# YufengJin/BundleSDF

Hardware: AMD Instinct MI355X
Metric: NeRF training rays/sec + ms/iter, 64-frame pool, 2048 rays/frame (higher is better)
Workload: dtype fp16 table+MLP (MFMA) / fp32 accumulate+Adam (amp)

## Files before the change

### bundlesdf_amd/csrc/field_step.hip

```cpp
#include <array>
#include <vector>

#include "field_core.h"
#include "field_host.h"

#pragma clang fp contract(off)

namespace nof {

constexpr int LOSS_ACC_COUNTERS = 136;
constexpr int LOSS_ACC_WORDS = 144;
constexpr int TREC = 12;
enum { TR_WSUM = 0, TR_NVALID, TR_LFS, TR_LEM, TR_LSDF, TR_CNT, TR_RACC = 8, TR_LFSR = 11 };
enum { TC_SIG = 1, TC_COL = 2, TC_CRCOL = 4, TC_CRSIG = 8 };
constexpr int LOSS_COPIES = 64, LOSS_SLOTS = 16, LOSS_FOLD_N = 13;
constexpr uint64_t LOSS_ZERO_WORDS = 16 + (uint64_t)LOSS_COPIES * LOSS_SLOTS;

template <int CTRL> __device__ __forceinline__ int dpp_i(int v) {
    return __builtin_amdgcn_update_dpp(0, v, CTRL, 0xf, 0xf, true);
}
#define DPP_ROW_SHL(n) (0x100 + (n))
#define DPP_ROW_SHR(n) (0x110 + (n))

constexpr uint32_t SLOT_EMPTY = 0xffffffffu;
// ... 545 lines not shown
__device__ __forceinline__ void stage_block(const FieldArgs &a, char *smem) {
    NOF_STAGE_FRAGS(TM, NFR, FR0, false, a, smem, (staged_bias<TM, NFR>(smem)));
    __syncthreads();
}

template <typename TM, int WPB, int WAVES, bool DBG>
__global__ __launch_bounds__(WPB * 64) __attribute__((amdgpu_waves_per_eu(WAVES, WAVES))) void k_colour(FieldArgs a_) {
    const FieldArgs a = step_args(a_);
    const int wave = threadIdx.x >> 6, lane = threadIdx.x & 63;
    const int n = lane & 31, h = lane >> 5;
    extern __shared__ __attribute__((aligned(16))) char smem[];
    stage_block<TM, COL_NFR, COL_FR0>(a, smem);
    const float *s_b = staged_bias<TM, COL_NFR>(smem);
    LdsWt<TM> W(reinterpret_cast<const TM *>(smem), lane, COL_FR0);
    const int n_col = __builtin_amdgcn_readfirstlane(a.n_tiles[1]);
    const int wg = __builtin_amdgcn_readfirstlane((int)blockIdx.x * WPB + wave);
    const int stride = gridDim.x * WPB;
    typedef typename FragT<TM>::T Frag;
    int cur = wg < n_col ? a.ctile_list[wg] : 0;
    int nxt = a.ctile_list[min(wg + stride, max(n_col - 1, 0))];
    Frag cin_n;
    frag_zero<TM>(cin_n);
    float z_n = 0.f;
    auto fetch = [&](int sid_first) {
        z_n = a.zbuf[(size_t)sid_first + n];
        cin_n = load_cin<TM>(a.tile_aux + (size_t)(sid_first >> 5) * TILE_AUX, lane);
    };
    if (wg < n_col) fetch(__builtin_amdgcn_readfirstlane(cur));
    __builtin_amdgcn_s_waitcnt(0x0f70);
    for (int li = wg; li < n_col; li += stride) {
        const int sid0 = __builtin_amdgcn_readfirstlane(cur);
        const int nn = a.ctile_list[min(li + 2 * stride, n_col - 1)];
        const int r = sid0 / a.S;
        const size_t slot = (size_t)(sid0 >> 5);
        const size_t sid = (size_t)sid0 + n;
        const RayCtx c = load_ray(a, r);
        const float z = z_n;
        const float w = bell_weight(a, c.depth, z);
        float p[3], x[3];
        const bool valid = sample_point(c, z, p, x);
        const bool front = z < c.depth - a.trunc;
        float wc = valid && w > 0.f ? w : 0.f;
        float wf = a.fs_rgb_w > 0.f && front && valid && c.rtype == 0 ? a.inv_3RS : 0.f;
        asm volatile("" : "+v"(wc), "+v"(wf));
        const Frag shf = sh_frag<TM>(c, h, a.n_ff);
        Acts<TM> A;
        float logit[3];
        W.fence();
        mlp_colour_net_cin<TM>(W, s_b, A, cin_n, shf, lane, logit);
        fetch(__builtin_amdgcn_readfirstlane(li + stride < n_col ? nxt : sid0));
        float rc[3], lf = 0.f;
#pragma unroll
        for (int cc = 0; cc < 3; ++cc) {
            const float sg = sigmoidf(logit[cc]);
            rc[cc] = wc * sg;
            lf += (sg - 1.f) * (sg - 1.f) * wf;
        }
        if constexpr (DBG) {
            if (h == 0) {
                float *o = a.dbg_raw + sid * 4;
                o[0] = logit[0]; o[1] = logit[1]; o[2] = logit[2];
            }
        }
        if constexpr (sizeof(TM) == 2) {
            reinterpret_cast<h8v *>(a.tile_aux + slot * TILE_AUX + 192)[lane] = shf;
            float vx, vy, vz;
            view_dir(c, vx, vy, vz);
            const float2 d = lane == 0 ? make_float2(c.vd[0], c.vd[1])
                                       : (lane == 1 ? make_float2(c.vd[2], vx) : make_float2(vy, vz));
            reinterpret_cast<float2 *>(a.tile_aux + slot * TILE_AUX + min(lane, 2))[1] = d;
        }
        float s0, s1, s2, sf;
        half_sums(h == 0 ? rc[0] : rc[1], s0, s1);
        half_sums(h == 0 ? rc[2] : lf, s2, sf);
        reinterpret_cast<float4 *>(a.rrec + slot * TREC)[2] = make_float4(s0, s1, s2, sf);
        cur = nxt;
        nxt = nn;
    }
}

__global__ __launch_bounds__(256) void k_ray_final(FieldArgs a_) {
    const FieldArgs a = step_args(a_);
    const int r = blockIdx.x * blockDim.x + threadIdx.x;
    const int lane = threadIdx.x & 63, wave = threadIdx.x >> 6;
    float v[10];
#pragma unroll
    for (int k = 0; k < 10; ++k) v[k] = 0.f;
    if (r < a.R) {
        const int ntiles = a.S / 32;
        float wtot = 0.f, nvalid = 0.f, lfs = 0.f, lem = 0.f, lsdf = 0.f, lfsr = 0.f;
        float racc[3] = {0.f, 0.f, 0.f};
        int csig = 0, ccol = 0, crcol = 0, crsig = 0;
#pragma unroll 4
        for (int t = 0; t < ntiles; ++t) {
            const size_t slot = (size_t)r * ntiles + t;
            const float4 *q = reinterpret_cast<const float4 *>(a.rrec + slot * TREC);
            const float4 q0 = q[0], q1 = q[1], q2 = q[2];
            const uint8_t fl = a.tile_bwd[slot];
            wtot += q0.x; nvalid += q0.y; lfs += q0.z; lem += q0.w; lsdf += q1.x;
            const int cnt = __float_as_int(q1.y);
            csig += cnt & TC_SIG; ccol += (cnt >> 1) & 1; crcol += (cnt >> 2) & 1; crsig += (cnt >> 3) & 1;
            if (fl == 1 || fl == 3) {
                racc[0] += q2.x; racc[1] += q2.y; racc[2] += q2.z; lfsr += q2.w;
            }
        }
        const float *cx = a.rctx + (size_t)r * RCTX;
        const float tgt[3] = {cx[3], cx[4], cx[5]};
        const int frame = __float_as_int(cx[23]), rtype = __float_as_int(cx[24]);
        const bool vray = nvalid > 0.f && rtype == 0;
        const float rw = vray ? (frame == 0 ? a.ffw : 1.f) : 0.f;
        float drgb[3], lr = 0.f, rgb[3];
#pragma unroll
        for (int cc = 0; cc < 3; ++cc) {
            rgb[cc] = racc[cc] / (wtot + 1e-10f);
            const float e = rgb[cc] - tgt[cc];
            drgb[cc] = a.rgb_w * 2.f * e * rw * a.inv_3R;
            lr += e * e * rw;
        }
        v[0] = a.rgb_w * lr * a.inv_3R;
        v[1] = lfs * rw;
        v[2] = lem * rw;
        v[3] = lsdf * rw;
        v[4] = nvalid;
        v[5] = lfsr * rw;
        v[6] = (float)csig; v[7] = (float)ccol; v[8] = (float)crcol; v[9] = (float)crsig;
        if (a.dbg_rgb) {
            a.dbg_rgb[r * 3] = rgb[0]; a.dbg_rgb[r * 3 + 1] = rgb[1]; a.dbg_rgb[r * 3 + 2] = rgb[2];
        }
        float4 *ra = reinterpret_cast<float4 *>(a.ray_aux + (size_t)r * RAY_AUX);
        ra[0] = make_float4(drgb[0], drgb[1], drgb[2], wtot);
        ra[1] = make_float4(rw, 0.f, 0.f, 0.f);
        float4 *rg = reinterpret_cast<float4 *>(a.ray_grad + (size_t)r * 12);
        rg[0] = make_float4(0.f, 0.f, 0.f, 0.f);
        rg[1] = make_float4(0.f, 0.f, 0.f, 0.f);
        rg[2] = make_float4(0.f, 0.f, 0.f, 0.f);
    }
    __shared__ float s_v[4][10];
#pragma unroll
    for (int k = 0; k < 10; ++k) {
        const float t = wave_sum(v[k]);
        if (lane == 0) s_v[wave][k] = t;
    }
    __syncthreads();
    if (threadIdx.x < 10) {
        const int k = threadIdx.x;
        const float t = s_v[0][k] + s_v[1][k] + s_v[2][k] + s_v[3][k];
        constexpr int slot[10] = {0, 1, 2, 3, 4, 10, 6, 7, 8, 9};
        if (t != 0.f && (k != 5 || a.fs_rgb_w > 0.f)) atomic_add_f32(loss_row(a, (int)blockIdx.x) + slot[k], t);
    }
}

constexpr int ENCODE_GROUP_SMALL = 2;

constexpr int COMPACT_PER_BLOCK = 4096;
__global__ __launch_bounds__(256) void k_compact(const uint8_t *__restrict__ flags, int n, int *__restrict__ list,
                                                 int *__restrict__ count, int per_block, int *__restrict__ clist) {
    __shared__ int s_wave[3][4];
    __shared__ int s_base[3];
    const int lane = threadIdx.x & 63, wave = threadIdx.x >> 6;
    const int fpt = per_block >> 8;
    const int b0 = blockIdx.x * per_block + threadIdx.x * fpt;
    uint8_t fl[16];
    if (fpt == 16 && b0 + 16 <= n) {
        const uint4 v = *reinterpret_cast<const uint4 *>(flags + b0);
        const uint32_t w[4] = {v.x, v.y, v.z, v.w};
#pragma unroll
        for (int k = 0; k < 16; ++k) fl[k] = (uint8_t)(w[k >> 2] >> (8 * (k & 3)));
    } else {
#pragma unroll
        for (int k = 0; k < 16; ++k) fl[k] = (k < fpt && b0 + k < n) ? flags[b0 + k] : 0;
    }
    int mine[3] = {0, 0, 0};
#pragma unroll
    for (int k = 0; k < 16; ++k) {
        mine[0] += fl[k] == 1;
        mine[1] += fl[k] == 2;
        mine[2] += (fl[k] == 1 || fl[k] == 3);
    }
    int pm[3] = {mine[0], mine[1], mine[2]};
#pragma unroll
    for (int o = 1; o < 64; o <<= 1) {
#pragma unroll
        for (int q = 0; q < 3; ++q) {
            const int u = __shfl_up(pm[q], o, 64);
            if (lane >= o) pm[q] += u;
        }
    }
    if (lane == 63) {
#pragma unroll
        for (int q = 0; q < 3; ++q) s_wave[q][wave] = pm[q];
    }
    __syncthreads();
    if (threadIdx.x < 3) {
        const int q = threadIdx.x;
        const int tot = s_wave[q][0] + s_wave[q][1] + s_wave[q][2] + s_wave[q][3];
        int *cnt = count + (q == 0 ? 0 : (q == 1 ? 2 : 1));
        s_base[q] = (tot && (q < 2 || clist)) ? atomicAdd(cnt, tot) : 0;
    }
    __syncthreads();
    int off[3];
#pragma unroll
    for (int q = 0; q < 3; ++q) {
        off[q] = s_base[q] + pm[q] - mine[q];
        for (int w = 0; w < wave; ++w) off[q] += s_wave[q][w];
    }
#pragma unroll
    for (int k = 0; k < 16; ++k) {
        const int i = b0 + k;
        if (fl[k] == 1) list[off[0]++] = i << 5;
        if (fl[k] == 2) list[n - 1 - off[1]++] = (i << 5) | (int)0x80000000;
        if (clist && (fl[k] == 1 || fl[k] == 3)) clist[off[2]++] = i << 5;
    }
}

__device__ __forceinline__ int bwd_entry(const FieldArgs &a, int li, int n_c, int cap) {
    return a.tile_sid[li < n_c ? li : cap - 1 - (li - n_c)];
}

#include "field_mlp_bwd.h"

__device__ __forceinline__ void loss_fold(const float *__restrict__ part, float *__restrict__ loss_acc, int k) {
    if (k >= LOSS_FOLD_N) return;
    constexpr int dst[LOSS_FOLD_N] = {0, 1, 2, 3, 4, 5, LOSS_ACC_COUNTERS, LOSS_ACC_COUNTERS + 1, LOSS_ACC_COUNTERS + 2,
                                      LOSS_ACC_COUNTERS + 3, LOSS_ACC_COUNTERS + 4, LOSS_ACC_COUNTERS + 5,
                                      LOSS_ACC_COUNTERS + 6};
    float s = 0.f;
    for (int c = 0; c < LOSS_COPIES; ++c) s += part[c * LOSS_SLOTS + k];
    loss_acc[dst[k]] += s;
}

__host__ __device__ constexpr uint32_t scatter_wave_words(uint32_t mask, int VW) {
    return (1 + VW) * (mask + 1) + 160;
}
template <typename TM, typename TT, bool F16V, int WAVES>
__global__ __launch_bounds__(256) __attribute__((amdgpu_num_sgpr(80), amdgpu_waves_per_eu(WAVES, 8))) void k_scatter(FieldArgs a_) {
    const FieldArgs a = step_args(a_);
    extern __shared__ __attribute__((aligned(16))) char smem[];
    const int lane = threadIdx.x & 63;
    const int wave = __builtin_amdgcn_readfirstlane((int)(threadIdx.x >> 6));
    if (blockIdx.x == 0 && wave == 0) loss_fold(a.loss_part, a.loss_acc, lane);
    const int bx = (a.xcd_order & 2) ? xcd_block(blockIdx.x, gridDim.x) : (int)blockIdx.x;
    const int lpw = a.scatter_lpw, ngrp = ((int)a.L + lpw - 1) / lpw;
    const int gw = __builtin_amdgcn_readfirstlane(bx * 4 + wave);
    const int r = __builtin_amdgcn_readfirstlane(gw / ngrp);
    if (r >= a.R || ABL(65536)) return;
    const int lv0 = __builtin_amdgcn_readfirstlane((gw - r * ngrp) * lpw);
    const int nlev = min(lpw, (int)a.L - lv0);
    const int ntiles = a.S / 32;
    const uint8_t *flags = a.tile_bwd + (size_t)r * ntiles;
    const uint8_t fl = lane < ntiles ? flags[lane] : (uint8_t)0;
    uint32_t gm = lane < ntiles ? a.tile_gmask[(size_t)r * ntiles + lane] : 0u;
    const bool tf = fl == 1 || fl == 2;
    if (!__any(tf) || ABL(131072)) return;
    gm = tf ? gm : 0u;
    const uint32_t mask = a.slot_mask;
    constexpr int VW = F16V ? 1 : 2;
    uint32_t *keys = reinterpret_cast<uint32_t *>(smem) + (size_t)wave * scatter_wave_words(mask, VW);
    uint32_t *vals = F16V ? keys + 1 : keys + mask + 1;
    uint16_t *slist = reinterpret_cast<uint16_t *>(keys + (1 + VW) * (mask + 1));
    if constexpr (F16V) {
        for (uint32_t s = lane; s <= mask; s += 64) reinterpret_cast<uint2 *>(keys)[s] = make_uint2(0xffffffffu, 0u);
    } else {
        for (uint32_t s = lane; s <= mask; s += 64) keys[s] = 0xffffffffu;
        for (uint32_t s = lane; s < VW * (mask + 1); s += 64) vals[s] = 0u;
    }
    if ABL(262144) return;
    float *g32 = (sizeof(TM) == 2) ? nullptr : a.grad_table;
    __half *g16 = (sizeof(TM) == 2) ? a.grad_table16 : nullptr;
    const RayCtx c = load_ray(a, r);
    int n_act = 0;
    for (int ch = 0; ch * 64 < a.S; ++ch) {
        const int s = 64 * ch + lane;
        const uint32_t m0 = (uint32_t)__builtin_amdgcn_readlane((int)gm, 2 * ch);
        const uint32_t m1 = 2 * ch + 1 < 64 ? (uint32_t)__builtin_amdgcn_readlane((int)gm, 2 * ch + 1) : 0u;
        const bool cand = s < a.S && (((lane < 32 ? m0 : m1) >> (s & 31)) & 1u);
        const uint64_t b = __ballot(cand);
        if (cand) slist[n_act + (int)__popcll(b & ((1ull << lane) - 1ull))] = (uint16_t)s;
        n_act += (int)__popcll(b);
    }
    n_act = __builtin_amdgcn_readfirstlane(n_act);
    if (n_act == 0) return;
    __builtin_amdgcn_fence(__ATOMIC_SEQ_CST, "wavefront");
    const int nch = (n_act + 63) / 64;
    float sgz[3] = {0.f, 0.f, 0.f}, sg[3] = {0.f, 0.f, 0.f};
    int n_flush = 0, n_direct = 0;
    if (!ABL(32)) {
        typedef typename std::conditional<sizeof(TM) == 2, uint32_t, float2>::type GPair;
        const size_t RS = (size_t)a.R * a.S;
        const int n_it = nlev * nch;
        auto issue = [&](int lv, int ch, float &z, GPair &g, uint32_t &prt) {
            const int j = 64 * ch + lane;
            const int sj_raw = (int)slist[j];
            const int sj = j < n_act ? sj_raw : 0;
            const size_t sid = (size_t)r * a.S + sj;
            prt = sj >= a.N_oct ? 1u : 0u;
            z = a.zbuf[sid];
            g = reinterpret_cast<const GPair *>(a.dfeat)[(size_t)lv * RS + sid];
        };
        float z_nx = 0.f;
        GPair g_nx{};
        uint32_t prt_nx = 0u;
        issue(lv0, 0, z_nx, g_nx, prt_nx);
        int lv = lv0, ch = 0, lv_n = lv0, ch_n = 0;
        for (int it = 0; it < n_it; ++it) {
            const float z = z_nx;
            const GPair gq = g_nx;
            const uint32_t part = prt_nx;
            if (++ch_n == nch) { ch_n = 0; ++lv_n; }
            issue(min(lv_n, (int)a.L - 1), ch_n, z_nx, g_nx, prt_nx);
            const bool member = 64 * ch + lane < n_act;
            float p[3], x[3], g0, g1;
            h2v g01;
            sample_point(load_ray<true>(a, r), z, p, x);
            if constexpr (sizeof(TM) == 2) {
                g01 = __builtin_bit_cast(h2v, gq);
                g0 = (float)g01[0];
                g1 = (float)g01[1];
            } else {
                g01 = h2v{(_Float16)0.f, (_Float16)0.f};
                g0 = gq.x;
                g1 = gq.y;
            }
            const bool act = member && (g0 != 0.f || g1 != 0.f);
            if (ABL(1 << 25)) {
                n_flush += __any(act) ? (int)__popcll(__ballot(act)) : 0;
                n_direct += (__any(act) && lane == 0) ? 64 : 0;
            }
            const bool skipq = ABL(ABL_SKIPQ(lv >> 2));
            if (__any(act) && !skipq) {
                const LevelInfo li = level_info_uniform(a, lv);
                const float x01[3] = {(x[0] + 1) / 2, (x[1] + 1) / 2, (x[2] + 1) / 2};
                float gx[3] = {0.f, 0.f, 0.f};
                backward_level<TT, F16V>(a, li, member, act, part, x01, g0, g1, g01, gx, lane, keys, vals, mask, g32, g16,
                                         n_direct);
#pragma unroll
                for (int i = 0; i < 3; ++i) {
                    sgz[i] = __builtin_fmaf(gx[i], z, sgz[i]);
                    sg[i] += gx[i];
                }
            }
            if (ch == nch - 1 && !ABL(1) && !ABL(1 << 22) && !skipq) {
                const int nfl = flush_table<F16V>(keys, vals, mask, lane, g32, g16, ABL(128));
                n_flush += nfl;
            }
            if (++ch == nch) { ch = 0; ++lv; }
        }
    }
    if (!a.no_dx) {
        float tz[3], t1[3];
#pragma unroll
        for (int i = 0; i < 3; ++i) {
            tz[i] = 0.5f * wave_sum(sgz[i]);
            t1[i] = 0.5f * wave_sum(sg[i]);
        }
        if (lane < 12) {
            const int i = lane >> 2, j = lane & 3;
            const float gzi = i == 0 ? tz[0] : (i == 1 ? tz[1] : tz[2]);
            const float g1i = i == 0 ? t1[0] : (i == 1 ? t1[1] : t1[2]);
            const float dj = j == 0 ? c.dir[0] : (j == 1 ? c.dir[1] : c.dir[2]);
            const float v = j < 3 ? gzi * dj : g1i;
            if (ngrp == 1) a.ray_grad[(size_t)r * 12 + lane] += v;
            else atomic_add_f32(a.ray_grad + (size_t)r * 12 + lane, v);
        }
    }
    if (!a.count_atomics || ABL(16384)) return;
    const float nf = (float)__builtin_amdgcn_readfirstlane(n_flush), nd = wave_sum((float)n_direct);
    float *cnt = a.loss_acc + 8 + 2 * (r & 63);
    if (lane == 0 && nf != 0.f) atomic_add_f32(cnt, nf);
    if (lane == 0 && nd != 0.f) atomic_add_f32(cnt + 1, nd);
}

__global__ __launch_bounds__(256) void k_quad_mirror(FieldArgs a) {
    __shared__ uint32_t s_off[16], s_rs[16], s_end[16];
    if (threadIdx.x < a.L) {
        const LevelInfo li = level_info(a, threadIdx.x);
        s_off[threadIdx.x] = li.off;
        s_rs[threadIdx.x] = li.res + 1;
        s_end[threadIdx.x] = level_dense(li.res + 1, li.hs) ? li.off + li.hs : 0u;
    }
    __syncthreads();
    uint32_t end = 0;
    for (int l = 0; l < (int)a.L && s_end[l]; ++l) end = s_end[l];
    const uint32_t *t = reinterpret_cast<const uint32_t *>(a.table);
    uint4 *quads = const_cast<uint4 *>(a.quads);
    int lv = 0;
    for (uint32_t i = blockIdx.x * 256u + threadIdx.x; i < end; i += gridDim.x * 256u) {
        while (lv + 1 < (int)a.L && s_off[lv + 1] <= i) ++lv;
        const uint32_t rs = s_rs[lv], hi = i + rs + 1;
        if (hi >= s_end[lv]) continue;
        quads[i] = make_uint4(t[i], t[i + 1], t[i + rs], t[hi]);
    }
}

__global__ void k_zero_i32(int *__restrict__ p, int n) {
    const int i = blockIdx.x * blockDim.x + threadIdx.x;
    if (i < n) p[i] = 0;
}

__global__ __launch_bounds__(256) void k_trace(const float *__restrict__ pool, const int32_t *__restrict__ ids, int R,
// ... 56 lines not shown
        bias[i - n_frag_elems] = k >= 0 ? mlp[k] : 0.f;
    }
}

constexpr int SAMPLE_BATCH_MAX = 4096;
__global__ __launch_bounds__(1024) void k_sample_batch(const int64_t *__restrict__ frame_start, int F,
                                                      int rays_per_frame, uint32_t seed, int32_t *__restrict__ ids,
                                                      const nof_step_params *__restrict__ sp) {
    if (sp) seed = sp->batch_seed;
    __shared__ float s_t[1024];
    const int f = blockIdx.x, t = threadIdx.x;
    const int k = rays_per_frame, m = k + 1;
    const int chunk = (m + 1023) / 1024;
    const int j0 = t * chunk, j1 = min(m, j0 + chunk);
    const int64_t lo = frame_start[f], cnt = frame_start[f + 1] - lo;
    float e[5];
    float run = 0.f;
#pragma unroll
    for (int q = 0; q < 5; ++q) {
        e[q] = 0.f;
        const int j = j0 + q;
        if (q < chunk && j < j1) {
            const uint32_t i = (uint32_t)(f * m + j);
            const uint32_t u = hash32(seed ^ hash32(i * 0x85EBCA6BU + 0x27D4EB2FU));
            e[q] = -__logf(((float)u + 0.5f) * 2.3283064e-10f);
            run += e[q];
        }
    }
    s_t[t] = run;
    __syncthreads();
    for (int off = 1; off < 1024; off <<= 1) {
        const float x = s_t[t] + (t >= off ? s_t[t - off] : 0.f);
        __syncthreads();
        s_t[t] = x;
        __syncthreads();
    }
    const float total = s_t[1023];
    float acc = t > 0 ? s_t[t - 1] : 0.f;
    const float scale = (float)cnt / total;
#pragma unroll
    for (int q = 0; q < 5; ++q) {
        const int j = j0 + q;
        if (q < chunk && j < min(j1, k)) {
            acc += e[q];
            int64_t id = (int64_t)(acc * scale);
            id = (id < 0 || cnt <= 0) ? 0 : (id >= cnt ? cnt - 1 : id);
            ids[(size_t)f * k + j] = (int32_t)(lo + id);
        }
    }
}

}

extern "C" int nof_trace_rays(const float *pool, const int32_t *ids, int32_t R, const float *tf, const uint8_t *occ,
                              int32_t N, int32_t Kmax, float near_sc, float far_sc, float trunc, float *rays_out,
                              float *intervals, float *totals, int32_t *counts, const nof_step_params *sp,
                              void *stream) {
    if (R <= 0) return NOF_OK;
    if (N <= 0 || Kmax <= 0) return nof::set_error(NOF_EINVAL, "trace_rays: bad N=%d Kmax=%d", N, Kmax);
    const int tb = R >= 65536 ? 256 : 64;
    hipLaunchKernelGGL(nof::k_trace, dim3(nof::div_up(R, tb)), dim3(tb), 0, (hipStream_t)stream, pool, ids, R, tf,
                       occ, N, Kmax, near_sc, far_sc, trunc, rays_out, intervals, totals, counts, sp,
                       (const int32_t *)nullptr);
    return nof::check_launch("trace_rays");
}

extern "C" int nof_trace_rays_epoch(const float *pool, const int32_t *perm, const int32_t *epoch_step0, int32_t R,
                                    const float *tf, const uint8_t *occ, int32_t N, int32_t Kmax, float near_sc,
                                    float far_sc, float trunc, float *rays_out, float *intervals, float *totals,
                                    int32_t *counts, const nof_step_params *sp, void *stream) {
    if (R <= 0) return NOF_OK;
    if (!perm || !epoch_step0 || !sp)
        return nof::set_error(NOF_EINVAL, "trace_rays_epoch: perm, epoch_step0 and the step block are required");
    if (N <= 0 || Kmax <= 0) return nof::set_error(NOF_EINVAL, "trace_rays_epoch: bad N=%d Kmax=%d", N, Kmax);
    const int tb = R >= 65536 ? 256 : 64;
    hipLaunchKernelGGL(nof::k_trace, dim3(nof::div_up(R, tb)), dim3(tb), 0, (hipStream_t)stream, pool, perm, R, tf,
                       occ, N, Kmax, near_sc, far_sc, trunc, rays_out, intervals, totals, counts, sp, epoch_step0);
    return nof::check_launch("trace_rays_epoch");
}

extern "C" int nof_pack_mlp(const float *mlp, const int32_t *idx, int32_t n_frag_elems, int32_t n_bias, void *frags,
                            float *bias, int mlp_dtype, void *stream) {
    const int n = n_frag_elems + n_bias;
    if (mlp_dtype == NOF_F16)
        hipLaunchKernelGGL(nof::k_pack_mlp<_Float16>, dim3(nof::div_up(n, 256)), dim3(256), 0, (hipStream_t)stream,
                           mlp, idx, n_frag_elems, n_bias, (_Float16 *)frags, bias);
    else
        hipLaunchKernelGGL(nof::k_pack_mlp<float>, dim3(nof::div_up(n, 256)), dim3(256), 0, (hipStream_t)stream, mlp,
                           idx, n_frag_elems, n_bias, (float *)frags, bias);
    return nof::check_launch("pack_mlp");
}

extern "C" int nof_sample_batch(const int64_t *frame_start, int32_t F, int32_t rays_per_frame, uint32_t seed,
                                int32_t *ids, const nof_step_params *sp, void *stream) {
    const int n = F * rays_per_frame;
    if (n <= 0) return NOF_OK;
    if (rays_per_frame > nof::SAMPLE_BATCH_MAX)
        return nof::set_error(NOF_EINVAL, "sample_batch: rays_per_frame %d > %d", rays_per_frame,
                              nof::SAMPLE_BATCH_MAX);
    hipLaunchKernelGGL(nof::k_sample_batch, dim3(F), dim3(1024), 0, (hipStream_t)stream, frame_start,
                       F, rays_per_frame, seed, ids, sp);
    return nof::check_launch("sample_batch");
}

namespace {
constexpr int N_FIELD_KERNELS = 4;
struct FieldTiming {
    bool on = false;
    std::vector<std::array<hipEvent_t, N_FIELD_KERNELS + 1>> sets;
    size_t used = 0;
};
FieldTiming g_timing;
hipEvent_t *timing_set() {
    if (!g_timing.on) return nullptr;
    if (g_timing.used == g_timing.sets.size()) {
        std::array<hipEvent_t, N_FIELD_KERNELS + 1> e{};
        for (auto &x : e)
            if (hipEventCreate(&x) != hipSuccess) return nullptr;
        g_timing.sets.push_back(e);
    }
    return g_timing.sets[g_timing.used++].data();
}
inline void mark(hipEvent_t *ev, int i, hipStream_t st) {
    if (ev) (void)hipEventRecord(ev[i], st);
}

template <typename TM, typename TT, bool DBG>
auto encode_kernel(int g) {
    return g == 4 ? nof::k_encode<TM, TT, 4, DBG> : (g == 2 ? nof::k_encode<TM, TT, 2, DBG> : nof::k_encode<TM, TT, 1, DBG>);
}

template <typename TM, typename TT, int WPB>
int launch_field(const nof::FieldArgs &a, int n_cu, hipStream_t st) {
    const int ntiles = a.S / 32;
    hipLaunchKernelGGL(nof::k_ray_ctx, dim3(nof::div_up(a.R, 256)), dim3(256), 0, st, a);
    hipEvent_t *ev = timing_set();
    mark(ev, 0, st);
    if (a.quads && !a.quads_ready)
        hipLaunchKernelGGL(nof::k_quad_mirror, dim3(nof::tile_blocks(a.n_rows, 256, n_cu, 8)), dim3(256), 0, st, a);
    const size_t elds = (size_t)8 * 64 * 8 * sizeof(TM) + 2 * 64 * sizeof(float) + 8 * 16 * 32;
    {
        const dim3 eg(nof::div_up((uint64_t)a.R * ntiles, 8));
        const bool dbg = a.dbg_z || a.dbg_valid || a.dbg_raw;
        hipLaunchKernelGGL((dbg ? encode_kernel<TM, TT, true>(a.encode_group) : encode_kernel<TM, TT, false>(a.encode_group)),
                           eg, dim3(512), elds, st, a);
    }
    int rc = nof::check_launch("field_step(encode)");
    if (rc) return rc;
    mark(ev, 1, st);
    {
        const int nflags = a.R * ntiles;
        const int per = a.compact_per > 0 ? a.compact_per : (nflags >= 262144 ? nof::COMPACT_PER_BLOCK : 512);
        hipLaunchKernelGGL(nof::k_compact, dim3(nof::div_up((uint64_t)nflags, per)), dim3(256), 0, st, a.tile_bwd,
                           nflags, a.tile_sid, a.n_tiles, per, a.ctile_list);
        rc = nof::check_launch("field_step(compact)");
        if (rc) return rc;
        constexpr int WPB_C = 4;
        const int nbc = std::max(1, nof::tile_blocks(nflags, 8, n_cu, 6));
        const size_t clds = nof::staged_bytes<TM, nof::COL_NFR>();
        hipLaunchKernelGGL((a.dbg_raw ? nof::k_colour<TM, WPB_C, 6, true> : nof::k_colour<TM, WPB_C, 6, false>), dim3(nbc),
                           dim3(WPB_C * 64), clds, st, a);
        rc = nof::check_launch("field_step(colour)");
        if (rc) return rc;
        hipLaunchKernelGGL(nof::k_ray_final, dim3(nof::div_up(a.R, 256)), dim3(256), 0, st, a);
        rc = nof::check_launch("field_step(ray_final)");
        if (rc) return rc;
    }
    mark(ev, 2, st);
    const size_t mlds = nof::staged_bytes<TM, nof::N_FRAGS>(false, 16 * sizeof(float));
    if constexpr (sizeof(TM) == 2) {
        const int64_t nt_all = (int64_t)a.R * ntiles;
        const bool blk = a.bwd_flush != 1;
        const int nbt = std::max(1, nof::tile_blocks(nt_all, blk ? 48 : 128, n_cu, 1));
        const size_t tl0 = nof::bwd_tr_lds(0, 8), tl1 = nof::bwd_tr_lds(1, 8);
        const auto tr0 = a.n_ff > 0 ? (blk ? nof::k_mlp_bwd_tr<8, 0, true, true> : nof::k_mlp_bwd_tr<8, 0, true>)
                                    : (blk ? nof::k_mlp_bwd_tr<8, 0, false, true> : nof::k_mlp_bwd_tr<8, 0>);
        hipLaunchKernelGGL(tr0, dim3(nbt), dim3(8 * 64), tl0, st, a);
        rc = nof::check_launch("field_step(mlp_bwd_tr0)");
        if (rc) return rc;
        hipLaunchKernelGGL((blk ? nof::k_mlp_bwd_tr<8, 1, false, true> : nof::k_mlp_bwd_tr<8, 1>), dim3(nbt), dim3(8 * 64), tl1, st, a);
        rc = nof::check_launch("field_step(mlp_bwd_tr1)");
        if (rc) return rc;
    } else {
        const int nbb = std::max(1, nof::tile_blocks((int64_t)a.R * ntiles, 64, n_cu, 2));
        hipLaunchKernelGGL((nof::k_mlp_bwd<TM, 4, 2, 0>), dim3(nbb), dim3(4 * 64), mlds, st, a);
        rc = nof::check_launch("field_step(mlp_bwd0)");
        if (rc) return rc;
        const int nb1 = std::min(nbb, n_cu);
        hipLaunchKernelGGL((a.n_ff > 0 ? nof::k_mlp_bwd<TM, 4, 1, 1, true> : nof::k_mlp_bwd<TM, 4, 1, 1>), dim3(nb1), dim3(4 * 64), mlds, st, a);
        rc = nof::check_launch("field_step(mlp_bwd)");
        if (rc) return rc;
    }
    mark(ev, 3, st);
    const int n_grp = ((int)a.L + a.scatter_lpw - 1) / a.scatter_lpw;
    const dim3 sg(nof::div_up((uint64_t)a.R * n_grp, 4));
    if constexpr (sizeof(TM) == 2) {
        const size_t lds = (size_t)4 * 4 * nof::scatter_wave_words(a.slot_mask, 1);
        hipLaunchKernelGGL((nof::k_scatter<TM, TT, true, 7>), sg, dim3(256), lds, st, a);
    } else {
        hipLaunchKernelGGL((nof::k_scatter<TM, TT, false, 1>), sg, dim3(256),
                           (size_t)4 * 4 * nof::scatter_wave_words(a.slot_mask, 2), st, a);
    }
    rc = nof::check_launch("field_step(scatter)");
    if (rc) return rc;
    mark(ev, 4, st);
    return NOF_OK;
}

struct FieldWorkspace : nof::Carver {
    void *feat, *dfeat;
    float *zbuf, *ray_aux, *rctx, *rrec;
    uint8_t *tile_bwd;
    int *tile_sid, *n_tiles, *ctile;
    float4 *tile_aux;
    uint32_t *gmask;
    uint64_t off[NOF_WS_SECTIONS] = {};
    template <int I, typename T> T *part(size_t count) {
        static_assert(I < NOF_WS_SECTIONS - 1, "a new section needs a larger NOF_WS_SECTIONS in include/nof.h");
        return off[I] = bytes, take<T>(count);
    }
    FieldWorkspace(void *base, int R, int S, int mlp_dtype) : Carver(base) {
        const size_t el = mlp_dtype == NOF_F16 ? 2 : 4, n = (size_t)R * S, nt = (size_t)R * (S / 32);
        feat = part<0, char>(n * 32 * el);
        dfeat = part<1, char>(n * 32 * el);
        zbuf = part<2, float>(n);
        tile_bwd = part<3, uint8_t>(nt);
        tile_sid = part<4, int>(nt);
        n_tiles = part<5, int>(nof::LOSS_ZERO_WORDS);
        ray_aux = part<6, float>((size_t)R * nof::RAY_AUX);
        tile_aux = part<7, float4>(nt * nof::TILE_AUX);
        rctx = part<8, float>((size_t)R * nof::RCTX);
        gmask = part<9, uint32_t>(nt);
        rrec = part<10, float>(nt * nof::TREC);
        ctile = part<11, int>(nt);
        off[NOF_WS_SECTIONS - 1] = bytes;
    }
};
bool quads_on(const nof_field_desc *d) {
    return d->table_quads && d->table_rows > 0 && d->mlp_dtype == NOF_F16 && d->table_dtype == NOF_F16 &&
           d->R >= (d->quads_min_rays > 0 ? d->quads_min_rays : 32768) && !ABL_HOST(d, 512);
}
}

extern "C" size_t nof_field_workspace_bytes(int32_t R, int32_t S, int32_t mlp_dtype) {
    return FieldWorkspace(nullptr, R, S, mlp_dtype).bytes;
}

extern "C" int nof_field_workspace_offsets(int32_t R, int32_t S, int32_t mlp_dtype, uint64_t *offsets, int32_t n) {
    if (R < 0 || S <= 0 || !offsets || n < NOF_WS_SECTIONS)
        return nof::set_error(NOF_EINVAL, "field_workspace_offsets: bad R=%d S=%d or n=%d < %d", R, S, n,
                              NOF_WS_SECTIONS);
    const FieldWorkspace w(nullptr, R, S, mlp_dtype);
    for (int i = 0; i < NOF_WS_SECTIONS; ++i) offsets[i] = w.off[i];
    return NOF_OK;
}

extern "C" size_t nof_field_desc_size(void) { return sizeof(nof_field_desc); }

extern "C" int nof_quad_mirror(const nof_field_desc *d, void *stream) {
    if (!d) return nof::set_error(NOF_EINVAL, "quad_mirror: desc is NULL");
    if (d->L > 16 || d->C != 2)
        return nof::set_error(NOF_EINVAL, "quad_mirror: needs C=2, L<=16 (got %u,%u)", d->C, d->L);
    if (d->R <= 0 || !quads_on(d)) return NOF_OK;
    nof::FieldArgs a{};
    a.table = d->table; a.levels = (const float4 *)d->levels; a.L = d->L;
    a.quads = (const uint4 *)d->table_quads; a.n_rows = (uint32_t)d->table_rows;
    hipLaunchKernelGGL(nof::k_quad_mirror, dim3(nof::tile_blocks(a.n_rows, 256, nof::cu_count(), 8)), dim3(256), 0,
                       (hipStream_t)stream, a);
    return nof::check_launch("quad_mirror");
}

extern "C" int nof_field_step(const nof_field_desc *d, void *stream) {
    if (!d) return nof::set_error(NOF_EINVAL, "field_step: desc is NULL");
    if (d->S % 32 != 0 || d->S > 320 || d->N_oct + d->N_dep != d->S)
        return nof::set_error(NOF_EINVAL, "field_step: S=%d must be N_oct+N_dep, a multiple of 32, <= 320", d->S);
    if (int rc = nof::check_geometry("field_step", d, false)) return rc;
    if (d->R <= 0) return NOF_OK;
    if (d->bwd_flush < 0 || d->bwd_flush > 2)
        return nof::set_error(NOF_EINVAL, "field_step: bwd_flush %d (0 by batch size, 1 per wave, 2 block)", d->bwd_flush);
    if (d->compact_per_block != 0 && (d->compact_per_block < 256 || d->compact_per_block > nof::COMPACT_PER_BLOCK ||
                                      d->compact_per_block % 256 != 0))
        return nof::set_error(NOF_EINVAL, "field_step: compact_per_block %d (0 by batch size, else a multiple of 256 "
                              "in [256, %d])", d->compact_per_block, nof::COMPACT_PER_BLOCK);
    if (d->encode_group != 0 && d->encode_group != 1 && d->encode_group != 2 && d->encode_group != 4)
        return nof::set_error(NOF_EINVAL, "field_step: encode_group %d (0 by batch size, or 1, 2, 4)", d->encode_group);
    if (int rc = nof::check_frame_features("field_step", d->n_ff, d->ff, d->grad_ff, true)) return rc;
    if (d->mlp_dtype == NOF_F16 && !d->grad_table16)
        return nof::set_error(NOF_EINVAL, "field_step: amp mode needs grad_table16 (fp16 table gradient)");
    if (d->ablate && !NOF_ABLATE)
        return nof::set_error(NOF_EINVAL, "field_step: ablate bits need a -DNOF_ABLATE=1 build (timing experiments only)");
    if (!d->workspace) return nof::set_error(NOF_EINVAL, "field_step: workspace is NULL (nof_field_workspace_bytes)");
    const int slots = d->scatter_slots ? d->scatter_slots : 512;
    if (slots < 64 || slots > 2048 || (slots & (slots - 1)))
        return nof::set_error(NOF_EINVAL, "field_step: scatter_slots must be a power of two in [64, 2048]");
    bool amp;
    if (int rc = nof::check_dtype_pair("field_step", d, amp)) return rc;

    nof::FieldArgs a;
    nof::fill_sampling(a, d);
    nof::fill_model(a, d);
    a.t_rand = d->t_rand; a.seed = d->seed; a.perturb = d->perturb;
    a.fs_sdf = d->fs_sdf; a.ffw = d->first_frame_weight;
    a.rgb_w = d->rgb_weight; a.fs_w = d->fs_weight; a.empty_w = d->empty_weight; a.trunc_w = d->trunc_weight;
    a.inv_3R = 1.0f / (3.0f * (float)d->R);
    a.inv_RS = 1.0f / ((float)d->R * (float)d->S);
    a.inv_3RS = 1.0f / (3.0f * (float)d->R * (float)d->S);
    a.xcd_order = d->xcd_order;
    a.no_dx = d->skip_pose_grad != 0;
    a.quads = quads_on(d) ? (const uint4 *)d->table_quads : nullptr;
    a.n_rows = (uint32_t)d->table_rows;
    a.quads_ready = d->quads_prebuilt != 0;
    {
        const int L = std::max(1, (int)d->L);
        const int want = d->R >= 196608 ? 16 : (d->R >= 32768 ? 8 : (d->R >= 8192 ? 4 : 2));
        a.scatter_lpw = std::max(1, std::min(L, d->scatter_levels_per_wave > 0 ? (int)d->scatter_levels_per_wave : want));
    }
    a.bwd_flush = d->bwd_flush;
    a.count_atomics = d->count_atomics != 0;
    a.compact_per = d->compact_per_block;
    a.encode_group = d->encode_group ? d->encode_group : (d->R >= 8192 ? 1 : nof::ENCODE_GROUP_SMALL);
    a.sp = d->step_params;
    a.fs_rgb_w = d->fs_rgb_weight;
    a.loss_scale = d->loss_scale; a.grad_ff = d->grad_ff;
    a.grad_table = d->grad_table; a.grad_mlp = d->grad_mlp;
    a.grad_table16 = (__half *)d->grad_table16;
    a.ray_grad = d->ray_grad; a.loss_acc = d->loss_acc; a.dbg_z = d->dbg_z; a.dbg_raw = d->dbg_raw;
    a.dbg_valid = d->dbg_valid; a.dbg_rgb = d->dbg_rgb; a.ablate = d->ablate;
    a.slot_mask = (uint32_t)slots - 1;
    const FieldWorkspace ws(d->workspace, d->R, d->S, d->mlp_dtype);
    a.feat = ws.feat; a.dfeat = ws.dfeat; a.zbuf = ws.zbuf; a.tile_bwd = ws.tile_bwd; a.tile_sid = ws.tile_sid;
    a.n_tiles = ws.n_tiles; a.loss_part = (float *)ws.n_tiles + 16;
    a.ray_aux = ws.ray_aux; a.tile_aux = ws.tile_aux; a.rctx = ws.rctx; a.tile_gmask = ws.gmask; a.rrec = ws.rrec;
    a.ctile_list = ws.ctile;

    hipStream_t st = (hipStream_t)stream;
    const int n_cu = nof::cu_count();
    return amp ? launch_field<_Float16, __half, 4>(a, n_cu, st) : launch_field<float, float, 4>(a, n_cu, st);
}

extern "C" int nof_field_timing(int32_t enable) {
    g_timing.on = enable != 0;
    g_timing.used = 0;
    return NOF_OK;
}

extern "C" int nof_field_timing_collect(float *ms_sum, int32_t n, int32_t *calls) {
    if (!ms_sum || n < N_FIELD_KERNELS) return nof::set_error(NOF_EINVAL, "field_timing_collect: need 4 floats");
    for (int k = 0; k < n; ++k) ms_sum[k] = 0.f;
    for (size_t i = 0; i < g_timing.used; ++i) {
        auto &e = g_timing.sets[i];
        if (hipEventSynchronize(e[N_FIELD_KERNELS]) != hipSuccess)
            return nof::set_error(NOF_ELAUNCH, "field_timing_collect: event sync failed");
        for (int k = 0; k < N_FIELD_KERNELS; ++k) {
            float ms = 0.f;
            if (hipEventElapsedTime(&ms, e[k], e[k + 1]) != hipSuccess)
                return nof::set_error(NOF_ELAUNCH, "field_timing_collect: elapsed time failed");
            ms_sum[k] += ms;
        }
    }
    if (calls) *calls = (int32_t)g_timing.used;
    g_timing.used = 0;
    return NOF_OK;
}
```

### bundlesdf_amd/fused.py

```python
import ctypes
import dataclasses
import gc
import math
import os

import numpy as np
import torch

from . import _lib
from . import exchange as EX
from . import mlp_layout as ML

_F32, _F16 = 0, 1
MAX_LEVEL_RES = 1023
QUADS_MIN_RAYS = 32768
MAX_POSE_FRAMES = 1024


def lr_at(cfg, global_step, base):
    n_iters = cfg["n_step"] + 1
    if global_step <= 10:
        return base
    last = 10 * ((global_step - 1) // 10)
    return base * (cfg["decay_rate"] ** (float(last) / n_iters))
# ... 692 lines not shown
                      workspace=torch.empty(int(_lib.lib().nof_render_workspace_bytes(n, S)), dtype=torch.uint8,
                                            device=d))
            self._render_buf = rb
        return rb

    @torch.no_grad()
    def render_rays(self, ids, global_step=None, samples=False, chunk=32768):
        cfg = self.cfg
        ids = torch.as_tensor(ids).to(self.dev).to(torch.int32).contiguous().view(-1)
        R = int(ids.numel())
        S = cfg["N_samples"] + cfg["N_samples_around_depth"]
        dev = self.dev
        out = {"rgb": torch.empty(R, 3, device=dev), "depth": torch.empty(R, device=dev)}
        if samples:
            out.update(z=torch.empty(R, S, device=dev), sdf=torch.empty(R, S, device=dev),
                       valid=torch.empty(R, S, dtype=torch.uint8, device=dev))
        if R > 0:
            chunk = max(1, int(chunk))
            L = _lib.lib()
            st = _lib.stream_of(self.P)
            self.wait_exchange()
            self._prologue()
            sc = cfg["sc_factor"]
            trunc = truncation(cfg, self.global_step if global_step is None else global_step)
            rb = self._render_buffers(min(chunk, R))
            for lo in range(0, R, chunk):
                n = min(chunk, R - lo)
                _lib.check(L.nof_trace_rays(_lib.ptr(self.pool), _lib.ctypes.c_void_p(ids.data_ptr() + 4 * lo), n,
                                            _lib.ptr(self.tf_buf), _lib.ptr(self.occ), self.Nocc, self.Kmax,
                                            cfg["near"] * sc, cfg["far"] * sc, trunc, _lib.ptr(rb["rays"]),
                                            _lib.ptr(rb["intervals"]), _lib.ptr(rb["totals"]), None, None, st),
                           "trace_rays")
                D = _lib.FieldDesc()
                D.R, D.L, D.C, D.D = n, self.L, self.C, 3
                D.table = (self.emb16 if self.amp else self.P).data_ptr()
                D.levels = self.levels.data_ptr()
                D.table_dtype = D.mlp_dtype = _F16 if self.amp else _F32
                D.rays, D.tf, D.intervals, D.totals = (rb["rays"].data_ptr(), self.tf_buf.data_ptr(),
                                                       rb["intervals"].data_ptr(), rb["totals"].data_ptr())
                D.Kmax, D.N_oct, D.N_dep, D.S = self.Kmax, cfg["N_samples"], cfg["N_samples_around_depth"], S
                D.near_sc, D.far_sc, D.trunc = cfg["near"] * sc, cfg["far"] * sc, trunc
                D.neg_trunc_ratio, D.sdf_lambda = cfg["neg_trunc_ratio"], cfg["sdf_lambda"]
                D.frags, D.bias = self.frags.data_ptr(), self.bias.data_ptr()
                D.n_ff = self.n_ff
                if self.n_ff:
                    D.ff = self.P.data_ptr() + 4 * self.feat_off
                O = _lib.RenderOut(rgb=out["rgb"].data_ptr() + 12 * lo, depth=out["depth"].data_ptr() + 4 * lo,
                                   workspace=rb["workspace"].data_ptr())
                if samples:
                    O.z, O.sdf = out["z"].data_ptr() + 4 * S * lo, out["sdf"].data_ptr() + 4 * S * lo
                    O.valid = out["valid"].data_ptr() + S * lo
                _lib.check(L.nof_render_rays(_lib.ctypes.byref(D), _lib.ctypes.byref(O), st), "render_rays")
        if samples:
            out["valid"] = out["valid"].bool()
        return out

    @torch.no_grad()
    def render_view(self, c2w, K, H, W, frame_id=0, step=None, max_steps=512, n_refine=8, pixels=None, chunk=65536,
                    stats=False):
        from .view import pixel_indices
        H, W = int(H), int(W)
        dev = self.dev
        pix = None if pixels is None else pixel_indices(H, W, pixels).to(torch.int32).to(dev).contiguous()
        n = H * W if pix is None else int(pix.numel())
        shape = (H, W) if pix is None else (n,)
        if step is None:
            step = 0.5 * truncation(self.cfg, self.global_step)
        out = {"t": torch.empty(n, device=dev), "depth": torch.empty(n, device=dev),
               "normal": torch.empty(n, 3, device=dev), "rgb": torch.empty(n, 3, device=dev),
               "hit": torch.empty(n, dtype=torch.uint8, device=dev)}
        if stats:
            out.update(index=torch.empty(n, dtype=torch.int32, device=dev),
                       tiles=torch.empty(n, dtype=torch.int32, device=dev))
        V = _lib.ViewDesc()
        V.c2w[:] = np.asarray(c2w, np.float64).astype(np.float32).reshape(16).tolist()
        V.K[:] = np.asarray(K, np.float64).astype(np.float32).reshape(9).tolist()
        V.H, V.W = H, W
        V.step, V.max_steps, V.n_refine = float(step), int(max_steps), int(n_refine)
        V.frame_id, V.n_frames = int(frame_id), self.F
        V.occ, V.occ_n = self.occ.data_ptr(), self.Nocc
        D = _lib.FieldDesc()
        D.L, D.C, D.D, D.Kmax = self.L, self.C, 3, self.Kmax
        D.table = (self.emb16 if self.amp else self.P).data_ptr()
        D.levels = self.levels.data_ptr()
        D.table_dtype = D.mlp_dtype = _F16 if self.amp else _F32
        D.frags, D.bias = self.frags.data_ptr(), self.bias.data_ptr()
        D.n_ff = self.n_ff
        if self.n_ff:
            D.ff = self.P.data_ptr() + 4 * self.feat_off
        if n > 0:
            self.wait_exchange()
            self.pack_mlp()
            chunk = max(1, min(int(chunk), 1 << 24))
            L = _lib.lib()
            st = _lib.stream_of(self.P)
            m_max = min(chunk, n)
            vb = getattr(self, "_view_ws", None)
            need = int(L.nof_render_view_workspace_bytes(m_max, self.Kmax))
            if vb is None or vb.numel() < need:
                vb = self._view_ws = torch.empty(need, dtype=torch.uint8, device=dev)
            for lo in range(0, n, chunk):
                m = min(chunk, n - lo)
                V.n, V.pixel0 = m, lo if pix is None else 0
                V.pixels = None if pix is None else pix.data_ptr() + 4 * lo
                O = _lib.ViewOut(t=out["t"].data_ptr() + 4 * lo, depth=out["depth"].data_ptr() + 4 * lo,
                                 normal=out["normal"].data_ptr() + 12 * lo, rgb=out["rgb"].data_ptr() + 12 * lo,
                                 hit=out["hit"].data_ptr() + lo, workspace=vb.data_ptr())
                if stats:
                    O.index, O.tiles = out["index"].data_ptr() + 4 * lo, out["tiles"].data_ptr() + 4 * lo
                _lib.check(L.nof_render_view(_lib.ctypes.byref(D), _lib.ctypes.byref(V), _lib.ctypes.byref(O), st),
                           "render_view")
        else:
            V.n = 0
            _lib.check(_lib.lib().nof_render_view(_lib.ctypes.byref(D), _lib.ctypes.byref(V),
                                                  _lib.ctypes.byref(_lib.ViewOut()), None), "render_view")
        out["hit"] = out["hit"].bool()
        return {k: v.reshape(*shape, *v.shape[1:]) for k, v in out.items()}

    def refresh_half_table(self):
        self.wait_exchange()
        if self.amp:
            _lib.check(_lib.lib().nof_to_half(_lib.ptr(self.P), _lib.ptr(self.emb16), self.n_emb,
                                              _lib.stream_of(self.P)), "to_half")
            self._shard_mirror()

    WS_SECTIONS = ("feat", "dfeat", "zbuf", "tile_bwd", "tile_sid", "n_tiles", "ray_aux", "tile_aux", "rctx", "gmask",
                   "rrec", "ctile", "total")

    def _ws_offsets(self):
        R = self._R
        S = self.cfg["N_samples"] + self.cfg["N_samples_around_depth"]
        o = np.zeros(len(self.WS_SECTIONS), np.uint64)
        _lib.check(_lib.lib().nof_field_workspace_offsets(R, S, _F16 if self.amp else _F32,
                                                          o.ctypes.data_as(ctypes.c_void_p), len(o)),
                   "field_workspace_offsets")
        offs = {k: int(v) for k, v in zip(self.WS_SECTIONS, o)}
        assert offs["total"] == self.workspace.numel()
        return offs, R * (S // 32)

    def n_tile_records(self):
        off = self._ws_offsets()[0]["n_tiles"]
        c = self.workspace[off:off + 12].view(torch.int32).tolist()
        return int(c[0] + c[2])

    def tile_lists(self):
        offs, nt = self._ws_offsets()
        cnt = self.workspace[offs["n_tiles"]:offs["n_tiles"] + 12].view(torch.int32).tolist()
        full = self.workspace[offs["tile_sid"]:offs["tile_sid"] + 4 * nt].view(torch.int32)
        bl = torch.cat([full[:cnt[0]], full[nt - cnt[2]:]])
        assert bool((full[:cnt[0]] >= 0).all()) and bool((full[nt - cnt[2]:] < 0).all()), "tile list halves mixed"
        cl = self.workspace[offs["ctile"]:offs["ctile"] + 4 * nt].view(torch.int32)[:cnt[1]]
        return torch.sort(bl)[0], torch.sort(cl)[0]

    def field_kernel_ms(self):
        torch.cuda.synchronize()
        out = [a.elapsed_time(b) for a, b in self.kernel_ms]
        self.kernel_ms = []
        return out

    def split(self, flat):
        d = {"embeddings": flat[:self.n_emb].view(-1, self.C)}
        o = self.mlp_off
        for k in ML.MLP_KEYS:
            n = int(np.prod(ML.shapes(self.n_in, self.n_ff)[k]))
            d[k] = flat[o:o + n].view(ML.shapes(self.n_in, self.n_ff)[k])
            o += n
        if self.n_ff:
            d["features"] = flat[self.feat_off:self.pose_off].view(self.F, self.n_ff)
        d["pose"] = flat[self.pose_off:].view(self.F, 6)
        return d
```

Measured before the change: 29.22 million.

## Compact active rays in k_compact so scatter waves only visit rays with backward tiles

```diff
diff --git a/bundlesdf_amd/csrc/field_step.hip b/bundlesdf_amd/csrc/field_step.hip
--- a/bundlesdf_amd/csrc/field_step.hip
+++ b/bundlesdf_amd/csrc/field_step.hip
@@ -721,10 +721,16 @@
 
 constexpr int ENCODE_GROUP_SMALL = 2;
 
+constexpr int SCATTER_LIST_MIN_RAYS = 65536;
+constexpr int SCATTER_LIST_BIT = 4;
+__device__ __forceinline__ int *ray_list_entry(float *rctx, int i) {
+    return reinterpret_cast<int *>(rctx) + (size_t)(i >> 2) * RCTX + 28 + (i & 3);
+}
 constexpr int COMPACT_PER_BLOCK = 4096;
 __global__ __launch_bounds__(256) void k_compact(const uint8_t *__restrict__ flags, int n, int *__restrict__ list,
-                                                 int *__restrict__ count, int per_block, int *__restrict__ clist) {
-    __shared__ int s_wave[3][4];
+                                                 int *__restrict__ count, int per_block, int *__restrict__ clist,
+                                                 int ntiles, float *__restrict__ rctx) {
+    __shared__ int s_wave[4][4];
     __shared__ int s_base[3];
     const int lane = threadIdx.x & 63, wave = threadIdx.x >> 6;
     const int fpt = per_block >> 8;
@@ -739,25 +745,38 @@
 #pragma unroll
         for (int k = 0; k < 16; ++k) fl[k] = (k < fpt && b0 + k < n) ? flags[b0 + k] : 0;
     }
-    int mine[3] = {0, 0, 0};
+    int mine[4] = {0, 0, 0, 0};
 #pragma unroll
     for (int k = 0; k < 16; ++k) {
         mine[0] += fl[k] == 1;
         mine[1] += fl[k] == 2;
         mine[2] += (fl[k] == 1 || fl[k] == 3);
     }
-    int pm[3] = {mine[0], mine[1], mine[2]};
+    uint32_t bw = 0, rl = 0;
+#pragma unroll
+    for (int k = 0; k < 16; ++k) bw |= (fl[k] == 1 || fl[k] == 2) ? 1u << k : 0u;
+    const int k0 = (ntiles - b0 % ntiles) % ntiles;
+    for (int k = k0; rctx && k < fpt && b0 + k < n; k += ntiles) {
+        bool any = (bw >> k) & ((1u << ntiles) - 1u);
+        for (int j = fpt - k; j < ntiles; ++j) {
+            const uint8_t f = flags[b0 + k + j];
+            any |= f == 1 || f == 2;
+        }
+        rl |= any ? 1u << k : 0u;
+    }
+    mine[3] = __popc(rl);
+    int pm[4] = {mine[0], mine[1], mine[2], mine[3]};
 #pragma unroll
     for (int o = 1; o < 64; o <<= 1) {
 #pragma unroll
-        for (int q = 0; q < 3; ++q) {
+        for (int q = 0; q < 4; ++q) {
             const int u = __shfl_up(pm[q], o, 64);
             if (lane >= o) pm[q] += u;
         }
     }
     if (lane == 63) {
 #pragma unroll
-        for (int q = 0; q < 3; ++q) s_wave[q][wave] = pm[q];
+        for (int q = 0; q < 4; ++q) s_wave[q][wave] = pm[q];
     }
     __syncthreads();
     if (threadIdx.x < 3) {
@@ -767,11 +786,23 @@
         s_base[q] = (tot && (q < 2 || clist)) ? atomicAdd(cnt, tot) : 0;
     }
     __syncthreads();
-    int off[3];
-#pragma unroll
-    for (int q = 0; q < 3; ++q) {
-        off[q] = s_base[q] + pm[q] - mine[q];
+    int off[4];
+#pragma unroll
+    for (int q = 0; q < 4; ++q) {
+        off[q] = (q < 3 ? s_base[q] : 0) + pm[q] - mine[q];
         for (int w = 0; w < wave; ++w) off[q] += s_wave[q][w];
+    }
+    if (rctx) {
+        const int blk0 = blockIdx.x * per_block;
+        const int seg0 = (blk0 + ntiles - 1) / ntiles;
+        const int seg1 = (min(blk0 + per_block, n) + ntiles - 1) / ntiles;
+        int slot = seg0 + off[3];
+        for (int ray = (b0 + k0) / ntiles; rl; rl &= rl - 1) {
+            const int k = __ffs(rl) - 1;
+            *ray_list_entry(rctx, slot++) = ray + (k - k0) / ntiles;
+        }
+        const int tot = s_wave[3][0] + s_wave[3][1] + s_wave[3][2] + s_wave[3][3];
+        for (int i = seg0 + tot + (int)threadIdx.x; i < seg1; i += 256) *ray_list_entry(rctx, i) = -1;
     }
 #pragma unroll
     for (int k = 0; k < 16; ++k) {
@@ -811,9 +842,14 @@
     const int bx = (a.xcd_order & 2) ? xcd_block(blockIdx.x, gridDim.x) : (int)blockIdx.x;
     const int lpw = a.scatter_lpw, ngrp = ((int)a.L + lpw - 1) / lpw;
     const int gw = __builtin_amdgcn_readfirstlane(bx * 4 + wave);
-    const int r = __builtin_amdgcn_readfirstlane(gw / ngrp);
-    if (r >= a.R || ABL(65536)) return;
-    const int lv0 = __builtin_amdgcn_readfirstlane((gw - r * ngrp) * lpw);
+    const int e = __builtin_amdgcn_readfirstlane(gw / ngrp);
+    if (e >= a.R || ABL(65536)) return;
+    int r = e;
+    if (a.xcd_order & SCATTER_LIST_BIT) {
+        r = (int)*(ConstU32)(size_t)ray_list_entry(a.rctx, e);
+        if ((uint32_t)r >= (uint32_t)a.R) return;
+    }
+    const int lv0 = __builtin_amdgcn_readfirstlane((gw - e * ngrp) * lpw);
     const int nlev = min(lpw, (int)a.L - lv0);
     const int ntiles = a.S / 32;
     const uint8_t *flags = a.tile_bwd + (size_t)r * ntiles;
@@ -1176,7 +1212,8 @@
         const int nflags = a.R * ntiles;
         const int per = a.compact_per > 0 ? a.compact_per : (nflags >= 262144 ? nof::COMPACT_PER_BLOCK : 512);
         hipLaunchKernelGGL(nof::k_compact, dim3(nof::div_up((uint64_t)nflags, per)), dim3(256), 0, st, a.tile_bwd,
-                           nflags, a.tile_sid, a.n_tiles, per, a.ctile_list);
+                           nflags, a.tile_sid, a.n_tiles, per, a.ctile_list, ntiles,
+                           (a.xcd_order & nof::SCATTER_LIST_BIT) ? a.rctx : nullptr);
         rc = nof::check_launch("field_step(compact)");
         if (rc) return rc;
         constexpr int WPB_C = 4;
@@ -1329,7 +1366,8 @@
     a.inv_3R = 1.0f / (3.0f * (float)d->R);
     a.inv_RS = 1.0f / ((float)d->R * (float)d->S);
     a.inv_3RS = 1.0f / (3.0f * (float)d->R * (float)d->S);
-    a.xcd_order = d->xcd_order;
+    a.xcd_order = (d->xcd_order & 3) |
+                  (((d->xcd_order & nof::SCATTER_LIST_BIT) || d->R >= nof::SCATTER_LIST_MIN_RAYS) ? nof::SCATTER_LIST_BIT : 0);
     a.no_dx = d->skip_pose_grad != 0;
     a.quads = quads_on(d) ? (const uint4 *)d->table_quads : nullptr;
     a.n_rows = (uint32_t)d->table_rows;
diff --git a/bundlesdf_amd/fused.py b/bundlesdf_amd/fused.py
--- a/bundlesdf_amd/fused.py
+++ b/bundlesdf_amd/fused.py
@@ -868,6 +868,12 @@
         cl = self.workspace[offs["ctile"]:offs["ctile"] + 4 * nt].view(torch.int32)[:cnt[1]]
         return torch.sort(bl)[0], torch.sort(cl)[0]
 
+    def ray_list(self):
+        offs, _ = self._ws_offsets()
+        rec = self.workspace[offs["rctx"]:offs["rctx"] + 128 * self._R].view(torch.int32).view(self._R, 32)
+        slots = rec[:, 28:32].reshape(-1)[:self._R]
+        return slots[slots >= 0].clone()
+
     def field_kernel_ms(self):
         torch.cuda.synchronize()
         out = [a.elapsed_time(b) for a, b in self.kernel_ms]
```

Result: no change. 29.85 million, median of 6 (+2.1%).
